# 1dayac/spades_for_blackbird

Hardware: AMD Instinct MI355X
Metric: distinct k-mers/sec (k=21, 150 bp synthetic reads, count only) (higher is better)
Workload: dtype u64

## Files before the change

spades_for_blackbird_amd/build.py:

```python
import os
import subprocess
import sys
from concurrent.futures import ThreadPoolExecutor

HERE = os.path.dirname(os.path.abspath(__file__))
CSRC = os.path.join(HERE, "csrc")
LIB = os.path.join(HERE, "libbbk.so")
SOURCES = ["primitives.hip", "msd.hip", "superk.hip", "reads.hip", "count.hip", "extindex.hip", "tipclip.hip", "atclip.hip", "readfilter.hip", "unitigs.hip", "unitigs_write.hip", "edgeprof.hip", "kmerprof.hip", "hamclust.hip", "kmerstat.hip", "group.hip"]
HEADERS = ["bbk_internal.h", "kmer_ops.h", "extwalk.h", "msd.h", "msd_part.h", "msd_bucket.h", "msd_narrow_a.h", "msd_stage_b.h", "accum.h", "arena.h", "unitigs.h", os.path.join("..", "..", "include", "bbk.h")]
ARCH = "gfx950"
FLAGS = ["-O3", "-std=c++17", "-fPIC", "--offload-arch=" + ARCH, "-fopenmp", "-Wall", "-Wno-unused-function"]


def _hipcc():
    for c in (os.environ.get("HIPCC"), "/opt/rocm/bin/hipcc", "hipcc"):
        if c and (os.path.isabs(c) and os.path.exists(c) or not os.path.isabs(c)):
            return c
    raise RuntimeError("hipcc not found")


def _stale(target, deps):
    if not os.path.exists(target):
        return True
    t = os.path.getmtime(target)
    return any(os.path.getmtime(d) > t for d in deps if os.path.exists(d))


def build(force=False, verbose=False, extra_flags=None, suffix=""):
    global LIB
    hipcc = _hipcc()
    extra_flags = list(extra_flags or [])
    lib = LIB.replace(".so", suffix + ".so") if suffix else LIB
    srcs = [s for s in SOURCES if os.path.exists(os.path.join(CSRC, s))]
    hdrs = [os.path.join(CSRC, h) for h in HEADERS]
    objs = []
    jobs = []
    for s in srcs:
        src = os.path.join(CSRC, s)
        obj = os.path.join(CSRC, s.replace(".hip", suffix + ".o"))
        objs.append(obj)
        if force or _stale(obj, [src] + hdrs):
            jobs.append([hipcc] + FLAGS + extra_flags + ["-x", "hip", "-c", src, "-o", obj])

    def run(cmd):
        if verbose:
            print(" ".join(cmd), flush=True)
        r = subprocess.run(cmd, capture_output=True, text=True)
        if r.returncode != 0:
            raise RuntimeError("build failed: %s\n%s\n%s" % (" ".join(cmd), r.stdout, r.stderr))
        if verbose and r.stderr.strip():
            print(r.stderr)

    with ThreadPoolExecutor(max_workers=4) as ex:
        list(ex.map(run, jobs))
    if jobs or force or _stale(lib, objs):
        run([hipcc, "-shared", "-fPIC", "--offload-arch=" + ARCH, "-fopenmp", "-o", lib] + objs)
    return lib


def _llvm_tool(name):
    import shutil
    cands = []
    hipcc = shutil.which(_hipcc()) or _hipcc()
    if os.path.isabs(hipcc):
        root = os.path.dirname(os.path.dirname(os.path.realpath(hipcc)))
        cands += [os.path.join(root, "lib", "llvm", "bin", name), os.path.join(root, "llvm", "bin", name)]
    cands += [os.path.join("/opt/rocm/lib/llvm/bin", name), shutil.which(name)]
    for c in cands:
        if c and os.path.exists(c):
            return c
    return None


def kernel_resources(objs=None):
    import re
    import shutil
    import tempfile
    objdump, readelf = _llvm_tool("llvm-objdump"), _llvm_tool("llvm-readelf")
    if not objdump or not readelf:
        return None
    objs = objs or [os.path.join(CSRC, s.replace(".hip", ".o")) for s in SOURCES]
    out = []
    for obj in objs:
        if not os.path.exists(obj):
            continue
        d = tempfile.mkdtemp(prefix="bbk_res_")
        try:
            local = os.path.join(d, os.path.basename(obj))
            shutil.copy(obj, local)
            r = subprocess.run([objdump, "--offloading", local], capture_output=True, text=True, cwd=d)
            if r.returncode != 0:
                raise RuntimeError("llvm-objdump --offloading %s failed (%d): %s" % (obj, r.returncode, r.stderr[-500:]))
            for f in os.listdir(d):
                if ARCH not in f:
                    continue
                rn = subprocess.run([readelf, "--notes", os.path.join(d, f)], capture_output=True, text=True)
                if rn.returncode != 0:
                    raise RuntimeError("llvm-readelf --notes failed (%d): %s" % (rn.returncode, rn.stderr[-500:]))
                notes = rn.stdout
                name = None
                vals = {}
                for line in notes.splitlines():
                    m = re.match(r"\s*\.name:\s+(\S+)", line)
                    if m:
                        if name:
                            out.append((os.path.basename(obj), name, vals.get("private_segment_fixed_size", 0),
                                        vals.get("sgpr_spill_count", 0), vals.get("vgpr_spill_count", 0)))
                        name, vals = m.group(1), {}
                        continue
                    m = re.match(r"\s*\.(private_segment_fixed_size|sgpr_spill_count|vgpr_spill_count):\s+(\d+)", line)
                    if m and name:
                        vals[m.group(1)] = int(m.group(2))
                if name:
                    out.append((os.path.basename(obj), name, vals.get("private_segment_fixed_size", 0),
                                vals.get("sgpr_spill_count", 0), vals.get("vgpr_spill_count", 0)))
        finally:
            shutil.rmtree(d, ignore_errors=True)
    return [r for r in out if r[1].startswith("_Z") or r[1].startswith("k_")]


def check_resources():
    res = kernel_resources()
    if res is None:
        print("warning: llvm-objdump / llvm-readelf not found: kernel resource check skipped", file=sys.stderr)
        return None
    if not res:
        raise RuntimeError("no kernel metadata found in the built objects (objects not built?)")
    bad = [r for r in res if r[2] != 0 or r[4] != 0]
    if bad:
        raise RuntimeError("kernels using scratch / spilling VGPRs:\n" +
                           "\n".join("  %s %s scratch=%d sgpr_spill=%d vgpr_spill=%d" % r for r in bad))
    return res


if __name__ == "__main__":
    extra = [a for a in sys.argv[1:] if a.startswith("-D")]
    suffix = next((a.split("=", 1)[1] for a in sys.argv[1:] if a.startswith("--suffix=")), "")
    print(build(force="--force" in sys.argv, verbose=True, extra_flags=extra, suffix=suffix))
    if not suffix:
        r = check_resources()
        if r is not None:
            print("%d kernels: no scratch, no VGPR spills (SGPR spills in %d)" % (len(r), sum(1 for x in r if x[3])))
```

spades_for_blackbird_amd/csrc/msd_stage_b.h:

```cpp
#pragma once

namespace bbk {

__global__ void k_bucket_base(const uint32_t *__restrict__ seg_nb2, const uint32_t *__restrict__ seg_bin, uint32_t nseg,
                              uint32_t nbuckets, int b1, int w0bits, uint64_t *__restrict__ base) {
    const uint32_t g = blockIdx.x * blockDim.x + threadIdx.x;
    if (g >= nbuckets) return;
    const uint32_t lo = last_le(seg_bin, nseg, g);
    const uint64_t P = 1ull << (32 - b1), nb = seg_nb2[lo], j = g - seg_bin[lo];
    const uint64_t p = lo * P + (j * P + nb - 1) / nb;
    base[g] = w0bits > 32 ? p << (w0bits - 32) : 0ull;
}

template <int NT, int ITEMS>
__global__ __launch_bounds__(NT) __attribute__((amdgpu_waves_per_eu(6, 6))) void k_bucket_dist_nb(const uint32_t *__restrict__ buf, const uint64_t *__restrict__ base,
                                                       BucketArgs A) {
    constexpr int CAP = NT * ITEMS;
    constexpr int NWAVES = NT / 64;
    constexpr int DB = DistBins<1, 0>::N;
    constexpr int BPT = DB / NT;
    extern __shared__ __attribute__((aligned(16))) unsigned char smem[];
    uint32_t *bins = reinterpret_cast<uint32_t *>(smem);
    uint32_t *scan_tmp = bins + DB;
    uint32_t *mm = scan_tmp + 32;
    uint32_t *skeys = mm + 2 * NWAVES;

    const int tid = threadIdx.x, lane = tid & 63, wave = tid >> 6;
    const uint32_t b = A.bucket_ids ? A.bucket_ids[blockIdx.x] : blockIdx.x;
    uint32_t start, n;
    bucket_range(A, b, &start, &n);
    if (n == 0) {
        if (tid == 0) A.dcount[b] = 0;
        return;
    }
    if (n > (uint32_t)CAP) {
        if (tid == 0) A.dcount[b] = 0xFFFFFFFFu;
        return;
    }
    for (uint32_t q = tid; q < (uint32_t)DB; q += NT) bins[q] = 0;
#ifdef BBK_PHASE_PROF
    unsigned long long t_prev = clock64();
#endif

    const uint64_t kbase = base[b];
    uint32_t keys[ITEMS];
#pragma unroll
    for (int i = 0; i < ITEMS; ++i) {
        const uint32_t p = (uint32_t)(i * NT + tid);
        keys[i] = buf[start + (p < n ? p : n - 1u)];
    }
    uint32_t mn = ~0u, mx = 0;
#pragma unroll
    for (int i = 0; i < ITEMS; ++i) {
        keys[i] -= (uint32_t)kbase;
        mn = keys[i] < mn ? keys[i] : mn;
        mx = keys[i] > mx ? keys[i] : mx;
    }
#pragma unroll
    for (int dd = 32; dd >= 1; dd >>= 1) {
        const uint32_t a = __shfl_xor(mn, dd, 64), c = __shfl_xor(mx, dd, 64);
        mn = a < mn ? a : mn;
        mx = c > mx ? c : mx;
    }
    if (lane == 0) {
        mm[2 * wave] = mn;
        mm[2 * wave + 1] = mx;
    }
    __syncthreads();
    mn = ~0u;
    mx = 0;
#pragma unroll
    for (int j = 0; j < NWAVES; ++j) {
        mn = mm[2 * j] < mn ? mm[2 * j] : mn;
        mx = mm[2 * j + 1] > mx ? mm[2 * j + 1] : mx;
    }
    BBK_PH(3, 0, t_prev);
    const uint32_t kmin = mn;
    const int rbits = 32 - __builtin_clz((mx - mn) | 1u);
    const int sh = rbits > DistBins<1, 0>::LOG ? rbits - DistBins<1, 0>::LOG : 0;

#pragma unroll
    for (int i = 0; i < ITEMS; ++i) {
        const uint32_t p = (uint32_t)(i * NT + tid);
        if (p < n) atomicAdd(&bins[(keys[i] - kmin) >> sh], 1u);
    }
    __syncthreads();
    BBK_PH(3, 1, t_prev);
    uint32_t c[BPT];
    uint32_t sum = 0;
    bool big = false;
#pragma unroll
    for (int q = 0; q < BPT; ++q) {
        c[q] = bins[tid * BPT + q];
        sum += c[q];
        big = big || c[q] > kDistMaxBin;
    }
    uint32_t incl = sum;
    incl = wave_scan_incl(incl);
    if (lane == 63) scan_tmp[wave] = incl;
    if (__syncthreads_or(big)) {
        if (tid == 0) A.dcount[b] = 0xFFFFFFFFu;
        return;
    }
    uint32_t first = incl - sum;
    for (int j = 0; j < wave; ++j) first += scan_tmp[j];
    {
        uint32_t ex = first;
#pragma unroll
        for (int q = 0; q < BPT; ++q) {
            bins[tid * BPT + q] = ex;
            ex += c[q];
        }
    }
    __syncthreads();
    BBK_PH(3, 2, t_prev);
    uint32_t at[ITEMS];
#pragma unroll
    for (int i = 0; i < ITEMS; ++i) {
        const uint32_t p = (uint32_t)(i * NT + tid);
        at[i] = 0xFFFFFFFFu;
        if (p < n) {
            const uint32_t pos = atomicAdd(&bins[(keys[i] - kmin) >> sh], 1u);
            skeys[pos] = keys[i];
            at[i] = pos;
        }
    }
    __syncthreads();
    BBK_PH(3, 3, t_prev);
    constexpr int RB = 4;
#pragma unroll
    for (int i0 = 0; i0 < ITEMS; i0 += RB) {
        uint32_t sb[RB], e[RB];
#pragma unroll
        for (int u = 0; u < RB; ++u) {
            const int i = i0 + u;
            sb[u] = e[u] = 0;
            if (i < ITEMS) {
                const uint32_t p = (uint32_t)(i * NT + tid);
                if (p < n) {
                    const uint32_t d = (keys[i] - kmin) >> sh;
                    sb[u] = d ? bins[d - 1] : 0u;
                    e[u] = bins[d];
                }
            }
        }
        uint32_t o[RB][4];
#pragma unroll
        for (int u = 0; u < RB; ++u) {
#pragma unroll
            for (int c4 = 0; c4 < 4; ++c4) {
                const uint32_t y = sb[u] + c4;
                o[u][c4] = skeys[y < e[u] ? y : (e[u] ? e[u] - 1u : 0u)];
            }
        }
#pragma unroll
        for (int u = 0; u < RB; ++u) {
            const int i = i0 + u;
            if (i < ITEMS) {
                const uint32_t p = (uint32_t)(i * NT + tid);
                if (p < n) {
                    uint32_t before = 0;
#pragma unroll
                    for (int c4 = 0; c4 < 4; ++c4) {
                        const uint32_t y = sb[u] + c4;
                        if (y < e[u]) before += (o[u][c4] < keys[i] || (o[u][c4] == keys[i] && y < at[i])) ? 1u : 0u;
                    }
                    for (uint32_t y = sb[u] + 4; y < e[u]; ++y) {
                        const uint32_t ok = skeys[y];
                        before += (ok < keys[i] || (ok == keys[i] && y < at[i])) ? 1u : 0u;
                    }
                    at[i] = sb[u] + before;
                }
            }
        }
    }
    __syncthreads();
    BBK_PH(3, 4, t_prev);
#pragma unroll
    for (int i = 0; i < ITEMS; ++i)
        if (at[i] != 0xFFFFFFFFu) skeys[at[i]] = keys[i];
    __syncthreads();
    BBK_PH(3, 5, t_prev);

    uint32_t ostart = A.out_off ? A.out_off[b] : start;
    const uint32_t p0 = (uint32_t)tid * ITEMS;
    const uint32_t prev = (p0 > 0 && p0 - 1 < n) ? skeys[p0 - 1] : 0u;
    uint32_t mine[ITEMS];
    uint32_t nheads = 0, headbits = 0;
#pragma unroll
    for (int i = 0; i < ITEMS; ++i) {
        mine[i] = 0;
        if (p0 + i < n) {
            mine[i] = skeys[p0 + i];
            const bool h = (i == 0) ? (p0 == 0 || mine[0] != prev) : mine[i] != mine[i - 1];
            if (h) {
                headbits |= 1u << i;
                ++nheads;
            }
        }
    }
    uint32_t excl, total;
    {
        uint32_t hincl = wave_scan_incl(nheads);
        __syncthreads();
        if (lane == 63) scan_tmp[wave] = hincl;
        __syncthreads();
        uint32_t wbase, tot;
        wave_totals<NWAVES>(scan_tmp, lane, wave, wbase, tot);
        excl = wbase + hincl - nheads;
        total = tot;
        asm volatile("" : "+v"(ostart));
    }
    int seg = (int)excl - 1;
#pragma unroll
    for (int i = 0; i < ITEMS; ++i)
        if (p0 + i < n && (headbits & (1u << i))) skeys[++seg] = mine[i];
    __syncthreads();
    uint64_t *dst = reinterpret_cast<uint64_t *>(A.sorted_keys) + ostart;
    for (uint32_t s = tid; s < total; s += NT) dst[s] = (kbase + skeys[s]) & A.strip_mask;
    if (tid == 0 && total != n) atomicOr(A.dup_flag, 1u);
    if (tid == 0) A.dcount[b] = total;
    BBK_PH(3, 6, t_prev);
#ifdef BBK_PHASE_PROF
    if (threadIdx.x == 0) atomicAdd(&g_phase[3][7], 1ull);
#endif
}

template <int NT, int ITEMS>
static size_t bucket_dist_nb_smem() {
    return sizeof(uint32_t) * (DistBins<1, 0>::N + 32 + 2 * (NT / 64) + (size_t)NT * ITEMS);
}

constexpr int kViewSpan = 64;

__device__ inline uint32_t view_bucket(const uint64_t *__restrict__ off, uint32_t lo, uint32_t hi, uint64_t c) {
    while (hi - lo > 1) {
        const uint32_t mid = (lo + hi) >> 1;
        if (off[mid] <= c) lo = mid;
        else hi = mid;
    }
    return lo;
}

__global__ void k_view_tile_desc(const uint64_t *__restrict__ off, uint32_t nbuckets, uint64_t D, uint32_t keys_per_tile,
                                 uint32_t ntiles, uint2 *__restrict__ desc) {
    const uint32_t t = blockIdx.x * blockDim.x + threadIdx.x;
    if (t >= ntiles) return;
    const uint64_t c0 = (uint64_t)t * keys_per_tile;
    const uint64_t c1 = (c0 + keys_per_tile < D ? c0 + keys_per_tile : D) - 1u;
    const uint32_t b0 = view_bucket(off, 0, nbuckets, c0);
    desc[t] = make_uint2(b0, view_bucket(off, b0, nbuckets, c1));
}

template <bool TAG>
__global__ __launch_bounds__(PartCfg<1>::THREADS) void k_part_view(const uint32_t *__restrict__ slots,
                                                                   const uint64_t *__restrict__ off,
                                                                   const uint16_t *__restrict__ seg,
                                                                   const uint2 *__restrict__ vdesc, uint32_t stride,
                                                                   int hb, TileMap M, PartLevel L,
                                                                   uint32_t *__restrict__ cursor,
                                                                   Key<1> *__restrict__ out) {
    constexpr int kItems = PartCfg<1>::ITEMS, kTile = PartCfg<1>::TILE, kThreads = PartCfg<1>::THREADS, MAXB = 512;
    extern __shared__ __attribute__((aligned(16))) unsigned char smem[];
    uint32_t *lhist = reinterpret_cast<uint32_t *>(smem);
    uint32_t *lstart = lhist + MAXB;
    uint32_t *goff = lstart + MAXB;
    uint32_t *scan_tmp = goff + MAXB;
    Key<1> *stage = reinterpret_cast<Key<1> *>(scan_tmp + 32);
    uint32_t *toff = reinterpret_cast<uint32_t *>(stage + kTile);
    uint16_t *tseg = reinterpret_cast<uint16_t *>(toff + kViewSpan);
    uint32_t *vals_unused = nullptr;

    const int tid = threadIdx.x;
    const TileInfo T = tile_info(M, L, blockIdx.x, (uint32_t)kTile);
    const uint32_t count = T.count, nb = T.nb;
    const uint2 d = vdesc[blockIdx.x];
    const uint32_t b0 = d.x, span = d.y - d.x + 1u;
    const bool staged = span <= (uint32_t)kViewSpan;
    for (uint32_t b = tid; b < nb; b += kThreads) lhist[b] = 0;
    if (staged && tid < (int)span) {
        toff[tid] = (uint32_t)off[b0 + tid];
        tseg[tid] = seg[b0 + tid];
    }
    __syncthreads();

    const uint32_t c0 = (uint32_t)(T.begin >> 1), nkeys = count >> 1;
    uint32_t lo[kItems / 2], sg[kItems / 2];
#pragma unroll
    for (int j = 0; j < kItems / 2; ++j) {
        const uint32_t cl = (uint32_t)(j * kThreads + tid);
        const uint32_t c = c0 + (cl < nkeys ? cl : nkeys - 1u);
        uint32_t b, base;
        if (staged) {
            uint32_t i = 0, hi = span;
            while (hi - i > 1) {
                const uint32_t mid = (i + hi) >> 1;
                if (toff[mid] <= c) i = mid;
                else hi = mid;
            }
            b = b0 + i;
            base = toff[i];
            sg[j] = tseg[i];
        } else {
            b = view_bucket(off, b0, d.y + 1u, c);
            base = (uint32_t)off[b];
            sg[j] = seg[b];
        }
        lo[j] = slots[(size_t)b * stride + (c - base)];
    }
    Key<1> keys[kItems];
    uint32_t binrank[kItems];
#pragma unroll
    for (int j = 0; j < kItems / 2; ++j) {
        Key<1> x, r;
        x.w[0] = nw_key(sg[j], lo[j], hb);
        r = kmer_rc<1>(x, M.expand_k);
        if (TAG) {
            x.w[0] |= __umul64hi(xxh3_64<1>(x), 16ull) << (2 * M.expand_k);
            r.w[0] |= __umul64hi(xxh3_64<1>(r), 16ull) << (2 * M.expand_k);
        }
        keys[2 * j] = x;
        keys[2 * j + 1] = r;
    }
#pragma unroll
    for (int i = 0; i < kItems; ++i) asm volatile("" : "+v"(keys[i].w[0]));
#pragma unroll
    for (int i = 0; i < kItems; ++i) {
        const uint32_t local = tile_local<1, kThreads>(i, tid);
        binrank[i] = 0xFFFFFFFFu;
        if (local < count) {
            uint32_t pfx = prefix_of<1>(keys[i], L.dmode, L.w0bits);
            if (select_prefix(pfx, L)) {
                const uint32_t b = bin_of(pfx, L, nb);
                const uint32_t rank = atomicAdd(&lhist[b], 1u);
                binrank[i] = (b << 16) | rank;
            }
        }
    }
    __syncthreads();
    uint32_t vals[kItems] = {};
    part_tail<1, kItems, kThreads, MAXB, false, false>(keys, vals, binrank, lhist, lstart, goff, scan_tmp, stage,
                                                       vals_unused, nb, T.gbin0, L, cursor, out, nullptr, 0, 0ull);
}

static size_t part_view_smem() {
    return part_smem(1, PartCfg<1>::TILE, false, false, true) + (size_t)kViewSpan * (4 + 2);
}

__global__ void k_view_recanon(const uint64_t *__restrict__ in, const uint32_t *__restrict__ seg_off,
                               const uint32_t *__restrict__ seg_size, int k, uint64_t *__restrict__ out, uint64_t cap,
                               uint32_t *__restrict__ count) {
    const uint32_t o = seg_off[blockIdx.x], n = seg_size[blockIdx.x];
    const uint64_t mask = (1ull << (2 * k)) - 1ull;
    const int lane = threadIdx.x & 63;
    for (uint32_t i0 = 0; i0 < n; i0 += blockDim.x) {
        const uint32_t i = i0 + threadIdx.x;
        Key<1> x;
        x.w[0] = 0;
        bool keep = false;
        if (i < n) {
            x.w[0] = in[o + i] & mask;
            keep = !kmer_less_nucl<1>(kmer_rc<1>(x, k), x);
        }
        const uint64_t bal = __ballot(keep);
        uint32_t base = 0;
        if (lane == 0 && bal) base = atomicAdd(count, (uint32_t)__popcll(bal));
        base = __shfl(base, 0);
        const uint64_t at = (uint64_t)base + __popcll(bal & ((1ull << lane) - 1ull));
        if (keep && at < cap) out[at] = x.w[0];
    }
}

constexpr int kLtThreads = 1024;
constexpr int kLt1Items = 14;
constexpr int kLt2Items = 12;

struct LtLds {
    uint32_t *lhist;
    uint2 *tab;
    uint32_t *lstart, *scan_tmp;
    unsigned long long *mark;
    uint16_t *mbase, *nz;
    uint32_t *stage;
};
template <int ITEMS>
__device__ __forceinline__ LtLds lt_lds(unsigned char *smem) {
    constexpr int MW = kLtThreads * ITEMS / 64;
    LtLds S;
    S.lhist = reinterpret_cast<uint32_t *>(smem);
    S.tab = reinterpret_cast<uint2 *>(smem);
    S.lstart = S.lhist + 2 * kMaxBins;
    S.scan_tmp = S.lstart + kMaxBins;
    S.mark = reinterpret_cast<unsigned long long *>(S.scan_tmp + 64);
    S.mbase = reinterpret_cast<uint16_t *>(S.mark + MW);
    S.nz = S.mbase + MW;
    S.stage = reinterpret_cast<uint32_t *>(S.nz + kMaxBins);
    return S;
}
static size_t lt_smem(int items, size_t more) {
    const size_t tile = (size_t)kLtThreads * items;
    return sizeof(uint32_t) * (3 * kMaxBins + 64) + (tile / 64) * (8 + 2) + (size_t)kMaxBins * 2 + tile * 4 + more;
}

__device__ inline uint64_t lt_tagged(uint32_t seg, uint32_t lo, int lobits, int k) {
    Key<1> x;
    x.w[0] = ((uint64_t)seg << lobits) | lo;
    return x.w[0] | (__umul64hi(xxh3_64<1>(x), 16ull) << (2 * k));
}

template <int ITEMS, class KeyOf>
__device__ __forceinline__ void lt_tail(const LtLds &S, const uint32_t (&lo)[ITEMS], const uint32_t (&bins)[ITEMS / 2],
                                        uint32_t nb, uint32_t *__restrict__ cur, uint64_t slot_end, uint32_t rec_or,
                                        const PartLevel &L, uint32_t *__restrict__ out, KeyOf key_of) {
    constexpr int NT = kLtThreads, MW = NT * ITEMS / 64;
    static_assert(ITEMS % 2 == 0 && ITEMS <= 32 && NT * ITEMS < 65536, "packed bins, one bit per item, 16-bit positions");
    const uint32_t tid = threadIdx.x;
    const int lane = tid & 63, wave = tid >> 6;
    const uint32_t c = tid < nb ? S.lhist[tid] : 0u;
    uint32_t incl = c;
    incl = wave_scan_incl(incl);
    const unsigned long long nzb = __ballot(c != 0);
    if (lane == 63) S.scan_tmp[wave] = incl | ((uint32_t)__popcll(nzb) << 16);
    __syncthreads();
    uint32_t before, total;
    wave_totals<NT / 64>(S.scan_tmp, lane, wave, before, total);
    const uint32_t staged = total & 0xFFFFu;
    const uint32_t ex = (before & 0xFFFFu) + incl - c;
    const uint32_t myr = (before >> 16) + (uint32_t)__popcll(nzb & ((1ull << lane) - 1ull));
    S.lstart[tid] = ex;
    uint32_t greserve = 0;
    if (c) {
        greserve = atomicAdd(cur, c);
        S.nz[myr] = (uint16_t)tid;
        atomicOr(&S.mark[ex >> 6], 1ull << (ex & 63u));
    }
    __syncthreads();
#pragma unroll
    for (int i = 0; i < ITEMS; ++i) {
        const uint32_t bin = (bins[i >> 1] >> (16 * (i & 1))) & 0xFFFFu;
        if (bin != 0xFFFFu) {
            const uint32_t pos = atomicAdd(&S.lstart[bin], 1u);
            S.stage[pos] = lo[i];
        }
    }
    asm volatile("" : "+v"(greserve));
    if (c) {
        const int64_t room = (int64_t)slot_end - (int64_t)greserve;
        S.tab[myr] = make_uint2(greserve - ex, (uint32_t)(int32_t)(room < -(int64_t)0x7FFF0000 ? -(int64_t)0x7FFF0000 : room) + ex);
    }
    if (wave == 0) {
        constexpr int WPL = (MW + 63) / 64;
        uint32_t pw[WPL], tot = 0;
#pragma unroll
        for (int j = 0; j < WPL; ++j) {
            const int idx = lane * WPL + j;
            pw[j] = tot;
            tot += idx < MW ? (uint32_t)__popcll(S.mark[idx]) : 0u;
        }
        uint32_t inc2 = tot;
        inc2 = wave_scan_incl(inc2);
        const uint32_t lb = inc2 - tot;
#pragma unroll
        for (int j = 0; j < WPL; ++j) {
            const int idx = lane * WPL + j;
            if (idx < MW) S.mbase[idx] = (uint16_t)(lb + pw[j]);
        }
    }
    __syncthreads();
    const unsigned long long upto = (2ull << lane) - 1ull;
    const unsigned long long *wmark = S.mark + wave;
    const uint16_t *wmbase = S.mbase + wave;
    uint32_t full = 0;
#pragma unroll
    for (int i = 0; i < ITEMS; ++i) {
        const uint32_t pos = (uint32_t)i * NT + tid;
        if (pos < staged) {
            const uint32_t r = (uint32_t)wmbase[i * (NT / 64)] + (uint32_t)__popcll(wmark[i * (NT / 64)] & upto) - 1u;
            unsigned long long e = reinterpret_cast<const unsigned long long *>(S.tab)[r];
            const uint32_t rec = S.stage[pos];
            asm volatile("" : "+v"(e));
            if ((int32_t)pos >= (int32_t)(uint32_t)(e >> 32)) full |= 1u << i;
            else out[(uint32_t)e + pos] = rec | rec_or;
        }
    }
    if (full) {
#pragma unroll 1
        for (int i = 0; i < ITEMS; ++i) {
            if ((full >> i) & 1u) {
                const uint32_t pos = (uint32_t)i * NT + tid;
                const uint32_t r = (uint32_t)wmbase[i * (NT / 64)] + (uint32_t)__popcll(wmark[i * (NT / 64)] & upto) - 1u;
                const uint32_t sp = atomicAdd(L.spill_count, 1u);
                if (sp < L.spill_cap) reinterpret_cast<uint64_t *>(L.spill_keys)[sp] = key_of((uint32_t)S.nz[r], S.stage[pos]);
            }
        }
    }
}

template <bool DENSE>
__global__ __launch_bounds__(kLtThreads) __attribute__((amdgpu_waves_per_eu(8, 8))) void k_part_view_lt(
    const uint32_t *__restrict__ slots, const uint64_t *__restrict__ off, const uint16_t *__restrict__ seg,
    const uint2 *__restrict__ vdesc, uint32_t stride, int hb, const uint64_t *__restrict__ dense, uint64_t nkeys_all, int k,
    PartLevel L, uint32_t *__restrict__ cursor, uint32_t *__restrict__ out) {
    constexpr int NT = kLtThreads, ITEMS = kLt1Items, KPT = NT * ITEMS / 2, MW = NT * ITEMS / 64;
    extern __shared__ __attribute__((aligned(16))) unsigned char smem[];
    const LtLds S = lt_lds<ITEMS>(smem);
    uint32_t *toff = S.stage + NT * ITEMS;
    uint16_t *tseg = reinterpret_cast<uint16_t *>(toff + kViewSpan);
    const uint32_t tid = threadIdx.x;
    uint32_t xcc = 0;
    if (L.xcd_shift) {
        asm volatile("s_getreg_b32 %0, hwreg(HW_REG_XCC_ID)" : "=s"(xcc));
        xcc &= (1u << L.xcd_shift) - 1u;
    }
    const int lobits = 2 * k - 10;
    const uint32_t lomask = lobits >= 32 ? 0xFFFFFFFFu : (1u << lobits) - 1u;
    const uint64_t c0 = (uint64_t)blockIdx.x * KPT;
    const uint64_t left = nkeys_all - c0;
    const uint32_t nkeys = left < (uint64_t)KPT ? (uint32_t)left : (uint32_t)KPT;
    uint32_t b0 = 0, span = 0;
    bool staged_tab = false;
    if (!DENSE) {
        const uint2 d = vdesc[blockIdx.x];
        b0 = d.x;
        span = d.y - d.x + 1u;
        staged_tab = span <= (uint32_t)kViewSpan;
        if (staged_tab && tid < span) {
            toff[tid] = (uint32_t)off[b0 + tid];
            tseg[tid] = seg[b0 + tid];
        }
    }
    S.lhist[tid] = 0;
    if (tid < 2 * MW) reinterpret_cast<uint32_t *>(S.mark)[tid] = 0u;
    __syncthreads();

    uint64_t x[ITEMS / 2];
    if (DENSE) {
#pragma unroll
        for (int j = 0; j < ITEMS / 2; ++j) {
            const uint32_t cl = (uint32_t)(j * NT) + tid;
            x[j] = dense[c0 + (cl < nkeys ? cl : nkeys - 1u)];
        }
    } else {
        uint32_t w[ITEMS / 2], sg[ITEMS / 2];
#pragma unroll
        for (int j = 0; j < ITEMS / 2; ++j) {
            const uint32_t cl = (uint32_t)(j * NT) + tid;
            const uint32_t c = (uint32_t)c0 + (cl < nkeys ? cl : nkeys - 1u);
            uint32_t b, base;
            if (staged_tab) {
                uint32_t i = 0, hi = span;
                while (hi - i > 1) {
                    const uint32_t mid = (i + hi) >> 1;
                    if (toff[mid] <= c) i = mid;
                    else hi = mid;
                }
                b = b0 + i;
                base = toff[i];
                sg[j] = tseg[i];
            } else {
                b = view_bucket(off, b0, b0 + span, c);
                base = (uint32_t)off[b];
                sg[j] = seg[b];
            }
            w[j] = slots[(size_t)b * stride + (c - base)];
        }
#pragma unroll
        for (int j = 0; j < ITEMS / 2; ++j) x[j] = nw_key(sg[j], w[j], hb);
    }
    uint32_t lo[ITEMS], bins[ITEMS / 2];
#pragma unroll
    for (int j = 0; j < ITEMS / 2; ++j) {
        Key<1> a;
        a.w[0] = x[j];
        const uint64_t r = kmer_rc<1>(a, k).w[0];
        const uint32_t ba = (uint32_t)(x[j] >> lobits), br = (uint32_t)(r >> lobits);
        lo[2 * j] = (uint32_t)x[j] & lomask;
        lo[2 * j + 1] = (uint32_t)r & lomask;
        bins[j] = 0xFFFFFFFFu;
        if ((uint32_t)(j * NT) + tid < nkeys) {
            bins[j] = ba | (br << 16);
            atomicAdd(&S.lhist[ba], 1u);
            atomicAdd(&S.lhist[br], 1u);
        }
    }
    __syncthreads();
    const uint64_t slot_end = (uint64_t)tid * L.slot_stride + (L.xcd_shift ? (uint64_t)(xcc + 1u) * L.sub_cap : (uint64_t)L.slot_cap);
    lt_tail<ITEMS>(S, lo, bins, (uint32_t)kMaxBins, &cursor[(tid << L.xcd_shift) + xcc], slot_end, 0u, L, out,
                   [&](uint32_t bin, uint32_t rec) { return lt_tagged(bin, rec, lobits, k); });
}

__global__ __launch_bounds__(kLtThreads) __attribute__((amdgpu_waves_per_eu(8, 8))) void k_part_lt2(
    const uint32_t *__restrict__ in, const uint4 *__restrict__ desc, int k, PartLevel L, uint32_t *__restrict__ cursor,
    uint32_t *__restrict__ out) {
    constexpr int NT = kLtThreads, ITEMS = kLt2Items, MW = NT * ITEMS / 64;
    extern __shared__ __attribute__((aligned(16))) unsigned char smem[];
    const LtLds S = lt_lds<ITEMS>(smem);
    const uint32_t tid = threadIdx.x;
    const uint4 d = desc[blockIdx.x];
    const uint32_t begin = d.x, count = d.y, nb = d.z & 0xFFFFu, sgm = d.z >> 16, gbin0 = d.w;
    if (count == 0) return;
    const int lobits = 2 * k - 10;
    const uint32_t nsub = nb >> 4;
    const uint64_t segbits = (uint64_t)sgm << lobits;
    S.lhist[tid] = 0;
    if (tid < 2 * MW) reinterpret_cast<uint32_t *>(S.mark)[tid] = 0u;
    __syncthreads();
    uint32_t lo[ITEMS], bins[ITEMS / 2];
#pragma unroll
    for (int i = 0; i < ITEMS; ++i) {
        const uint32_t local = (uint32_t)i * NT + tid;
        lo[i] = in[begin + (local < count ? local : count - 1u)];
    }
#pragma unroll
    for (int i = 0; i < ITEMS; ++i) asm volatile("" : "+v"(lo[i]));
#pragma unroll
    for (int i = 0; i < ITEMS; ++i) {
        Key<1> x;
        x.w[0] = segbits | lo[i];
        const uint32_t tag = (uint32_t)__umul64hi(xxh3_64<1>(x), 16ull);
        const uint32_t b = tag * nsub + __umulhi(lo[i] << (32 - lobits), nsub);
        const bool valid = (uint32_t)i * NT + tid < count;
        if (valid) atomicAdd(&S.lhist[b], 1u);
        const uint32_t b16 = valid ? b : 0xFFFFu;
        if (i & 1) bins[i >> 1] |= b16 << 16;
        else bins[i >> 1] = b16;
    }
    __syncthreads();
    const uint64_t slot_end = (uint64_t)(gbin0 + tid) * L.slot_stride + L.slot_cap;
    lt_tail<ITEMS>(S, lo, bins, nb, &cursor[gbin0 + tid], slot_end, (uint32_t)segbits, L, out,
                   [&](uint32_t, uint32_t rec) { return lt_tagged(sgm, rec, lobits, k); });
}

__global__ void k_bucket_base_lt(const uint32_t *__restrict__ seg_nb2, const uint32_t *__restrict__ seg_bin, uint32_t nseg,
                                 uint32_t nbuckets, int lobits, int k, uint64_t *__restrict__ base,
                                 uint32_t *__restrict__ perm) {
    const uint32_t g = blockIdx.x * blockDim.x + threadIdx.x;
    if (g >= nbuckets) return;
    const uint32_t lo = last_le(seg_bin, nseg, g);
    const uint32_t nsub = seg_nb2[lo] >> 4, r = g - seg_bin[lo], tag = r / nsub, j = r - tag * nsub;
    const uint64_t q = (((uint64_t)j << lobits) + nsub - 1u) / nsub;
    base[g] = ((uint64_t)tag << (2 * k)) | ((uint64_t)lo << lobits) | q;
    perm[g] = tag * (nbuckets >> 4) + (seg_bin[lo] >> 4) + j;
}

__global__ void k_lt_fill_perm(const uint32_t *__restrict__ cursor, const uint32_t *__restrict__ perm, uint32_t n,
                               uint32_t stride, uint32_t cap, uint32_t *__restrict__ fill) {
    const uint32_t g = blockIdx.x * blockDim.x + threadIdx.x;
    if (g >= n) return;
    const uint32_t c = cursor[g] - g * stride;
    fill[perm[g]] = c < cap ? c : cap;
}

__global__ void k_lt_unperm(const uint64_t *__restrict__ scanned, const uint32_t *__restrict__ perm, uint32_t n,
                            uint32_t *__restrict__ out_off) {
    const uint32_t g = blockIdx.x * blockDim.x + threadIdx.x;
    if (g < n) out_off[g] = (uint32_t)scanned[perm[g]];
}

__global__ void k_view_recanon_lt(const uint32_t *__restrict__ in, const uint32_t *__restrict__ seg_off,
                                  const uint32_t *__restrict__ seg_size, int sub_shift, int k, uint64_t *__restrict__ out,
                                  uint64_t cap, uint32_t *__restrict__ count) {
    const uint32_t o = seg_off[blockIdx.x], n = seg_size[blockIdx.x];
    const uint64_t segbits = (uint64_t)(blockIdx.x >> sub_shift) << (2 * k - 10);
    const int lane = threadIdx.x & 63;
    for (uint32_t i0 = 0; i0 < n; i0 += blockDim.x) {
        const uint32_t i = i0 + threadIdx.x;
        Key<1> x;
        x.w[0] = 0;
        bool keep = false;
        if (i < n) {
            x.w[0] = segbits | in[o + i];
            keep = !kmer_less_nucl<1>(kmer_rc<1>(x, k), x);
        }
        const uint64_t bal = __ballot(keep);
        uint32_t base = 0;
        if (lane == 0 && bal) base = atomicAdd(count, (uint32_t)__popcll(bal));
        base = __shfl(base, 0);
        const uint64_t at = (uint64_t)base + __popcll(bal & ((1ull << lane) - 1ull));
        if (keep && at < cap) out[at] = x.w[0];
    }
}

void BucketView::materialise(bbk_ctx *ctx) {
    if (!live()) return;
    keys.alloc(n() * 8 + 16);
    if (nbuckets) {
        KernelTimer t(ctx, "compact", (double)D * (4 + 8));
        hipLaunchKernelGGL(k_compact_narrow<false>, dim3((unsigned)(((uint64_t)nbuckets * 64 + 255) / 256)), dim3(256), 0,
                           ctx->stream, slots.as<uint32_t>(), nullptr, dcount.as<uint32_t>(), off.as<uint64_t>(), nbuckets,
                           stride, seg.as<uint16_t>(), hb, keys.as<uint64_t>(), nullptr);
        check_launch("compact");
    }
    if (n_extra)
        BBK_HIP(bbk::copy_async(keys.as<uint64_t>() + D, extra.p, n_extra * 8, hipMemcpyDeviceToDevice, ctx->stream));
    stream_wait(ctx);
    release_slots();
}

}
```

Measured before the change: 29.59 billion.

## Drop block-wide dedup compaction in bucket sort tail and skip empty rows

The bucket sort tail no longer runs a head-flag scan and in-LDS compaction. It writes every sorted key straight out, detects adjacent duplicates per element and raises the dup flag with one atomic per wave. Loops now skip item rows beyond the bucket's occupancy, the rank-refinement unroll drops from 4 to 2, and the waves-per-EU hint rises from 6 to 8. Output is now undeduplicated with dcount set to n, so correctness depends on a downstream path that handles the dup flag; if duplicates are common, that fallback could add cost.

Result: faster. 30.68 billion (median of 6 runs) (+3.7%).

```diff
diff --git a/spades_for_blackbird_amd/build.py b/spades_for_blackbird_amd/build.py
--- a/spades_for_blackbird_amd/build.py
+++ b/spades_for_blackbird_amd/build.py
@@ -7,7 +7,7 @@
 CSRC = os.path.join(HERE, "csrc")
 LIB = os.path.join(HERE, "libbbk.so")
 SOURCES = ["primitives.hip", "msd.hip", "superk.hip", "reads.hip", "count.hip", "extindex.hip", "tipclip.hip", "atclip.hip", "readfilter.hip", "unitigs.hip", "unitigs_write.hip", "edgeprof.hip", "kmerprof.hip", "hamclust.hip", "kmerstat.hip", "group.hip"]
-HEADERS = ["bbk_internal.h", "kmer_ops.h", "extwalk.h", "msd.h", "msd_part.h", "msd_bucket.h", "msd_narrow_a.h", "msd_stage_b.h", "accum.h", "arena.h", "unitigs.h", os.path.join("..", "..", "include", "bbk.h")]
+HEADERS = ["bbk_internal.h", "kmer_ops.h", "extwalk.h", "msd.h", "msd_part.h", "msd_bucket.h", "msd_narrow_a.h", "msd_stage_b.h", "msd_bucket_tail.h", "accum.h", "arena.h", "unitigs.h", os.path.join("..", "..", "include", "bbk.h")]
 ARCH = "gfx950"
 FLAGS = ["-O3", "-std=c++17", "-fPIC", "--offload-arch=" + ARCH, "-fopenmp", "-Wall", "-Wno-unused-function"]
 
diff --git a/spades_for_blackbird_amd/csrc/msd_bucket_tail.h b/spades_for_blackbird_amd/csrc/msd_bucket_tail.h
--- /dev/null
+++ b/spades_for_blackbird_amd/csrc/msd_bucket_tail.h
@@ -0,0 +1,21 @@
+#pragma once
+
+#include <cstdint>
+
+#if defined(__HIPCC__) || defined(__CUDACC__)
+#define BBK_HOST_DEVICE __host__ __device__
+#else
+#define BBK_HOST_DEVICE
+#endif
+
+namespace bbk {
+
+BBK_HOST_DEVICE inline bool dist_tail_at(const uint32_t *sorted, uint32_t s, uint64_t base, uint64_t mask, uint64_t *dst) {
+    const uint32_t x = sorted[s];
+    dst[s] = (base + x) & mask;
+    return s > 0 && sorted[s - 1] == x;
+}
+
+BBK_HOST_DEVICE inline uint32_t bucket_rows(uint32_t n, uint32_t nt) { return (n + nt - 1u) / nt; }
+
+}
diff --git a/spades_for_blackbird_amd/csrc/msd_stage_b.h b/spades_for_blackbird_amd/csrc/msd_stage_b.h
--- a/spades_for_blackbird_amd/csrc/msd_stage_b.h
+++ b/spades_for_blackbird_amd/csrc/msd_stage_b.h
@@ -1,4 +1,6 @@
 #pragma once
+
+#include "msd_bucket_tail.h"
 
 namespace bbk {
 
@@ -13,7 +15,7 @@
 }
 
 template <int NT, int ITEMS>
-__global__ __launch_bounds__(NT) __attribute__((amdgpu_waves_per_eu(6, 6))) void k_bucket_dist_nb(const uint32_t *__restrict__ buf, const uint64_t *__restrict__ base,
+__global__ __launch_bounds__(NT) __attribute__((amdgpu_waves_per_eu(8, 8))) void k_bucket_dist_nb(const uint32_t *__restrict__ buf, const uint64_t *__restrict__ base,
                                                        BucketArgs A) {
     constexpr int CAP = NT * ITEMS;
     constexpr int NWAVES = NT / 64;
@@ -42,19 +44,24 @@
     unsigned long long t_prev = clock64();
 #endif
 
+    const uint32_t rows = bucket_rows(n, NT);
     const uint64_t kbase = base[b];
     uint32_t keys[ITEMS];
 #pragma unroll
     for (int i = 0; i < ITEMS; ++i) {
-        const uint32_t p = (uint32_t)(i * NT + tid);
-        keys[i] = buf[start + (p < n ? p : n - 1u)];
+        if ((uint32_t)i < rows) {
+            const uint32_t p = (uint32_t)(i * NT + tid);
+            keys[i] = buf[start + (p < n ? p : n - 1u)];
+        }
     }
     uint32_t mn = ~0u, mx = 0;
 #pragma unroll
     for (int i = 0; i < ITEMS; ++i) {
-        keys[i] -= (uint32_t)kbase;
-        mn = keys[i] < mn ? keys[i] : mn;
-        mx = keys[i] > mx ? keys[i] : mx;
+        if ((uint32_t)i < rows) {
+            keys[i] -= (uint32_t)kbase;
+            mn = keys[i] < mn ? keys[i] : mn;
+            mx = keys[i] > mx ? keys[i] : mx;
+        }
     }
 #pragma unroll
     for (int dd = 32; dd >= 1; dd >>= 1) {
@@ -81,8 +88,10 @@
 
 #pragma unroll
     for (int i = 0; i < ITEMS; ++i) {
-        const uint32_t p = (uint32_t)(i * NT + tid);
-        if (p < n) atomicAdd(&bins[(keys[i] - kmin) >> sh], 1u);
+        if ((uint32_t)i < rows) {
+            const uint32_t p = (uint32_t)(i * NT + tid);
+            if (p < n) atomicAdd(&bins[(keys[i] - kmin) >> sh], 1u);
+        }
     }
     __syncthreads();
     BBK_PH(3, 1, t_prev);
@@ -117,59 +126,62 @@
     uint32_t at[ITEMS];
 #pragma unroll
     for (int i = 0; i < ITEMS; ++i) {
-        const uint32_t p = (uint32_t)(i * NT + tid);
-        at[i] = 0xFFFFFFFFu;
-        if (p < n) {
-            const uint32_t pos = atomicAdd(&bins[(keys[i] - kmin) >> sh], 1u);
-            skeys[pos] = keys[i];
-            at[i] = pos;
+        if ((uint32_t)i < rows) {
+            const uint32_t p = (uint32_t)(i * NT + tid);
+            if (p < n) {
+                const uint32_t pos = atomicAdd(&bins[(keys[i] - kmin) >> sh], 1u);
+                skeys[pos] = keys[i];
+                at[i] = pos;
+            }
         }
     }
     __syncthreads();
     BBK_PH(3, 3, t_prev);
-    constexpr int RB = 4;
+    constexpr int RB = 2;
 #pragma unroll
     for (int i0 = 0; i0 < ITEMS; i0 += RB) {
-        uint32_t sb[RB], e[RB];
-#pragma unroll
-        for (int u = 0; u < RB; ++u) {
-            const int i = i0 + u;
-            sb[u] = e[u] = 0;
-            if (i < ITEMS) {
-                const uint32_t p = (uint32_t)(i * NT + tid);
-                if (p < n) {
-                    const uint32_t d = (keys[i] - kmin) >> sh;
-                    sb[u] = d ? bins[d - 1] : 0u;
-                    e[u] = bins[d];
+        if ((uint32_t)i0 < rows) {
+            uint32_t sb[RB], e[RB];
+#pragma unroll
+            for (int u = 0; u < RB; ++u) {
+                const int i = i0 + u;
+                sb[u] = e[u] = 0;
+                if (i < ITEMS) {
+                    const uint32_t p = (uint32_t)(i * NT + tid);
+                    if (p < n) {
+                        const uint32_t d = (keys[i] - kmin) >> sh;
+                        sb[u] = d ? bins[d - 1] : 0u;
+                        e[u] = bins[d];
+                    }
                 }
             }
-        }
-        uint32_t o[RB][4];
-#pragma unroll
-        for (int u = 0; u < RB; ++u) {
-#pragma unroll
-            for (int c4 = 0; c4 < 4; ++c4) {
-                const uint32_t y = sb[u] + c4;
-                o[u][c4] = skeys[y < e[u] ? y : (e[u] ? e[u] - 1u : 0u)];
-            }
-        }
-#pragma unroll
-        for (int u = 0; u < RB; ++u) {
-            const int i = i0 + u;
-            if (i < ITEMS) {
-                const uint32_t p = (uint32_t)(i * NT + tid);
-                if (p < n) {
-                    uint32_t before = 0;
-#pragma unroll
-                    for (int c4 = 0; c4 < 4; ++c4) {
-                        const uint32_t y = sb[u] + c4;
-                        if (y < e[u]) before += (o[u][c4] < keys[i] || (o[u][c4] == keys[i] && y < at[i])) ? 1u : 0u;
+            uint32_t o[RB][4];
+#pragma unroll
+            for (int u = 0; u < RB; ++u) {
+#pragma unroll
+                for (int c4 = 0; c4 < 4; ++c4) {
+                    const uint32_t y = sb[u] + c4;
+                    o[u][c4] = skeys[y < e[u] ? y : (e[u] ? e[u] - 1u : 0u)];
+                }
+            }
+#pragma unroll
+            for (int u = 0; u < RB; ++u) {
+                const int i = i0 + u;
+                if (i < ITEMS) {
+                    const uint32_t p = (uint32_t)(i * NT + tid);
+                    if (p < n) {
+                        uint32_t before = 0;
+#pragma unroll
+                        for (int c4 = 0; c4 < 4; ++c4) {
+                            const uint32_t y = sb[u] + c4;
+                            if (y < e[u]) before += (o[u][c4] < keys[i] || (o[u][c4] == keys[i] && y < at[i])) ? 1u : 0u;
+                        }
+                        for (uint32_t y = sb[u] + 4; y < e[u]; ++y) {
+                            const uint32_t ok = skeys[y];
+                            before += (ok < keys[i] || (ok == keys[i] && y < at[i])) ? 1u : 0u;
+                        }
+                        at[i] = sb[u] + before;
                     }
-                    for (uint32_t y = sb[u] + 4; y < e[u]; ++y) {
-                        const uint32_t ok = skeys[y];
-                        before += (ok < keys[i] || (ok == keys[i] && y < at[i])) ? 1u : 0u;
-                    }
-                    at[i] = sb[u] + before;
                 }
             }
         }
@@ -177,49 +189,28 @@
     __syncthreads();
     BBK_PH(3, 4, t_prev);
 #pragma unroll
-    for (int i = 0; i < ITEMS; ++i)
-        if (at[i] != 0xFFFFFFFFu) skeys[at[i]] = keys[i];
+    for (int i = 0; i < ITEMS; ++i) {
+        if ((uint32_t)i < rows) {
+            const uint32_t p = (uint32_t)(i * NT + tid);
+            if (p < n) skeys[at[i]] = keys[i];
+        }
+    }
+    uint32_t ostart = A.out_off ? A.out_off[b] : start;
     __syncthreads();
     BBK_PH(3, 5, t_prev);
-
-    uint32_t ostart = A.out_off ? A.out_off[b] : start;
-    const uint32_t p0 = (uint32_t)tid * ITEMS;
-    const uint32_t prev = (p0 > 0 && p0 - 1 < n) ? skeys[p0 - 1] : 0u;
-    uint32_t mine[ITEMS];
-    uint32_t nheads = 0, headbits = 0;
-#pragma unroll
-    for (int i = 0; i < ITEMS; ++i) {
-        mine[i] = 0;
-        if (p0 + i < n) {
-            mine[i] = skeys[p0 + i];
-            const bool h = (i == 0) ? (p0 == 0 || mine[0] != prev) : mine[i] != mine[i - 1];
-            if (h) {
-                headbits |= 1u << i;
-                ++nheads;
-            }
-        }
-    }
-    uint32_t excl, total;
-    {
-        uint32_t hincl = wave_scan_incl(nheads);
-        __syncthreads();
-        if (lane == 63) scan_tmp[wave] = hincl;
-        __syncthreads();
-        uint32_t wbase, tot;
-        wave_totals<NWAVES>(scan_tmp, lane, wave, wbase, tot);
-        excl = wbase + hincl - nheads;
-        total = tot;
-        asm volatile("" : "+v"(ostart));
-    }
-    int seg = (int)excl - 1;
-#pragma unroll
-    for (int i = 0; i < ITEMS; ++i)
-        if (p0 + i < n && (headbits & (1u << i))) skeys[++seg] = mine[i];
-    __syncthreads();
+    asm volatile("" : "+v"(ostart));
+
     uint64_t *dst = reinterpret_cast<uint64_t *>(A.sorted_keys) + ostart;
-    for (uint32_t s = tid; s < total; s += NT) dst[s] = (kbase + skeys[s]) & A.strip_mask;
-    if (tid == 0 && total != n) atomicOr(A.dup_flag, 1u);
-    if (tid == 0) A.dcount[b] = total;
+    bool dup = false;
+#pragma unroll
+    for (int i = 0; i < ITEMS; ++i) {
+        if ((uint32_t)i < rows) {
+            const uint32_t s = (uint32_t)(i * NT + tid);
+            if (s < n) dup = dist_tail_at(skeys, s, kbase, A.strip_mask, dst) || dup;
+        }
+    }
+    if (__any(dup) && lane == 0) atomicOr(A.dup_flag, 1u);
+    if (tid == 0) A.dcount[b] = n;
     BBK_PH(3, 6, t_prev);
 #ifdef BBK_PHASE_PROF
     if (threadIdx.x == 0) atomicAdd(&g_phase[3][7], 1ull);
```
